# Rita-zi/WavTokenizer

Measured on AMD Instinct MI355X. Metric: audio-seconds/sec encode+decode, 24 kHz 3 s clips, higher is better.
Workload: dtype f32 (split-f16 x3 products)

## Files before the change

### include/wavtokenizer_amd.h

```cpp
#ifndef WAVTOKENIZER_AMD_H
#define WAVTOKENIZER_AMD_H

#include <stddef.h>
#include <stdint.h>

#ifdef __cplusplus
extern "C" {
#endif

typedef enum {
    WT_OK = 0,
    WT_ERR_INVALID = -1,
    WT_ERR_MISSING_TENSOR = -2,
    WT_ERR_SHAPE = -3,
    WT_ERR_HIP = -4,
    WT_ERR_NOT_INITED = -5,
    WT_ERR_RANGE = -6,
    WT_ERR_LSTM_SYNC = -7,
    WT_ERR_INDEX = -8
} wt_status;

enum wt_status_bits {
    WT_STATUS_BIT_LSTM = 1,
    WT_STATUS_BIT_RANGE = 2,
// ... 33 lines not shown
    WT_PLAN_DECODE_MIXED = 5,
    WT_PLAN_DECODE_CODES = 6,
    WT_PLAN_DECODE_CODES_MIXED = 7,
    WT_PLAN_QUANTIZE = 8
} wt_plan_kind;

enum {
    WT_PLAN_FLAG_KEEP_STAGES = 1,
    WT_PLAN_FLAG_UNFUSED = 16,
    WT_PLAN_FLAG_STEP_LSTM = 4,
    WT_PLAN_FLAG_GRAPH = 8,
    WT_PLAN_FLAG_FP32_GEMM = 2,
    WT_PLAN_FLAG_RANGE_REPORT = 32,
    WT_PLAN_FLAG_MIXED_LENGTH = 64,
    WT_PLAN_FLAG_F16_GEMM = 128,
    WT_PLAN_FLAG_RVQ = 256
};

enum wt_range_site {
    WT_SITE_ENCODER = 0,
    WT_SITE_BB_EMBED = 1,
    WT_SITE_RES0 = 2, WT_SITE_RES1 = 3,
    WT_SITE_ATTN = 4,
    WT_SITE_RES2 = 5, WT_SITE_RES3 = 6,
    WT_SITE_CNX0 = 7,
    WT_SITE_HEAD = 40,
    WT_SITE_SEANET_DECODER = 41
};

const char* wt_last_error(void);
// ... 140 lines not shown
    const float* R;
    const float* gamma;
    float* C;
    float* C2;
    uint32_t* status;
    const int32_t* mix_geom;
} wt_gemm_desc;
typedef struct {
    int32_t BM, BN, waves_m, waves_n, stages, ks, prod, staged, bias_cache, G, tiles;
} wt_launch_form;
size_t wt_gemm_probe_workspace_bytes(const wt_gemm_desc* d);
int wt_gemm_probe(const wt_gemm_desc* d, wt_launch_form* form, void* workspace, void* stream);

enum { WT_OP_GN_APPLY = 0, WT_OP_GN_STATS = 1, WT_OP_ROWNORM = 2, WT_OP_SOFTMAX = 3, WT_OP_ISTFT_OLA = 4, WT_OP_CONV_FIRST = 5,
       WT_OP_CONV_LAST = 6, WT_OP_TRANSPOSE = 7, WT_OP_CONVTR = 8, WT_OP_ROW_SUMSQ = 9, WT_OP_S32_AMAX = 10,
       WT_OP_CODE_ROWS = 12 };
enum { WT_OPK_GN_TILE = 1, WT_OPK_GN_CHUNK = 2, WT_OPK_GN_STATS = 3, WT_OPK_ROWNORM = 4, WT_OPK_DWCONV_LN = 5,
       WT_OPK_SOFTMAX_REG = 6, WT_OPK_SOFTMAX_RMW = 7, WT_OPK_ISTFT_OLA = 8, WT_OPK_CONV_FIRST = 9, WT_OPK_CONV_LAST32 = 10,
       WT_OPK_CONV_LAST = 11, WT_OPK_TRANSPOSE = 12, WT_OPK_CONVTR = 13, WT_OPK_ROW_SUMSQ = 14, WT_OPK_S32_AMAX = 15,
       WT_OPK_TRANSPOSE_MIXED = 16, WT_OPK_GN_MIXED = 17, WT_OPK_DWCONV_LN_MIXED = 18, WT_OPK_SOFTMAX_REG_MIXED = 19,
       WT_OPK_SOFTMAX_RMW_MIXED = 20, WT_OPK_ISTFT_OLA_MIXED = 21,
       WT_OPK_CODE_ROWS = 22, WT_OPK_CODE_ROWS_MIXED = 23 };
typedef struct {
    int32_t size;
    int32_t op;
    int32_t B, L, C;
    int32_t groups, mode, flag, out_s32;
    int32_t ld, k, stride, Cout, n_fft, hop, Kq;
    float eps;
    int64_t n;
    const void* x;
    const void *p0, *p1, *p2, *p3, *p4, *p5;
    void *y, *y2, *y3;
    uint32_t* status;
    const int32_t* lengths;
} wt_op_desc;
typedef struct {
// ... 248 lines not shown
```

### wavtokenizer_amd/_capi.py

```python
from __future__ import annotations

import ctypes
import os
from ctypes import POINTER, c_char_p, c_float, c_int32, c_int64, c_size_t, c_void_p

_HERE = os.path.dirname(os.path.abspath(__file__))
LIB_PATH = os.environ.get("WAVTOK_HIP_LIB") or os.path.join(_HERE, "libwavtok_hip.so")

EXPORTS = [
    "wt_last_error", "wt_version", "wt_model_create", "wt_model_destroy", "wt_model_export_bytes", "wt_model_export", "wt_packed_info", "wt_packed_verify", "wt_packed_bytes",
    "wt_model_create_packed", "wt_model_hop", "wt_model_weight_bytes",
    "wt_plan_create", "wt_plan_create_ex", "wt_plan_range_sites", "wt_plan_range_report", "wt_model_persistent_lstm", "wt_device_info", "wt_plan_destroy", "wt_plan_workspace_bytes", "wt_plan_frames", "wt_plan_num_launches", "wt_plan_graph_replays",
    "wt_plan_find_buffer", "wt_plan_buffer_info", "wt_plan_buffer_name", "wt_plan_status", "wt_plan_num_steps", "wt_plan_step_name",
    "wt_plan_set_timing", "wt_plan_read_timing", "wt_model_split_ok", "wt_model_status", "wt_model_take_bad_codes", "wt_encode", "wt_codes_to_features",
    "wt_decode", "wt_seanet_decode", "wt_head", "wt_unit_run", "wt_sconv1d", "wt_linear", "wt_conv1d_s32", "wt_vq_workspace_bytes",
    "wt_vq_nearest", "wt_vq_nearest_f32", "wt_resblock", "wt_resblock_down", "wt_gemm_probe_workspace_bytes", "wt_gemm_probe", "wt_op_probe",
    "wt_resampler_create", "wt_resampler_destroy", "wt_resampler_out_length", "wt_convert_audio", "wt_pcm16",
    "wt_linear_overlap_add", "wt_encode_mixed", "wt_plan_min_clip_length", "wt_sconv_geometry", "wt_decode_mixed",
    "wt_resblock_probe", "wt_geometry_words", "wt_geometry_probe", "wt_lstm_probe_workspace_bytes", "wt_lstm_probe",
    "wt_decode_codes", "wt_decode_codes_mixed", "wt_ingest_workspace_bytes", "wt_ingest", "wt_codes_unpack",
    "wt_emit_workspace_bytes", "wt_emit", "wt_vq_probe", "wt_overlap_add_ragged_workspace_bytes", "wt_overlap_add_ragged",
    "wt_model_weight_count", "wt_model_weight_info", "wt_split_probe",
    "wt_encode_rvq", "wt_encode_rvq_mixed", "wt_quantize", "wt_vq_residual_probe", "wt_model_codebook_tables",
    "wt_mel_create", "wt_mel_destroy", "wt_mel_frames", "wt_mel_tables", "wt_mel_workspace_bytes", "wt_mel_spectrogram", "wt_mel_distance",
# ... 4 lines not shown
]

WT_PLAN_ENCODE, WT_PLAN_DECODE, WT_PLAN_SEANET_DECODER, WT_PLAN_HEAD, WT_PLAN_UNIT_LSTM = 0, 1, 2, 3, 4
WT_PLAN_DECODE_MIXED = 5
WT_PLAN_DECODE_CODES, WT_PLAN_DECODE_CODES_MIXED = 6, 7
WT_PLAN_QUANTIZE = 8
WT_PLAN_FLAG_KEEP_STAGES = 1
WT_PLAN_FLAG_FP32_GEMM = 2
WT_PLAN_FLAG_F16_GEMM = 128
WT_PLAN_FLAG_STEP_LSTM = 4
WT_PLAN_FLAG_GRAPH = 8
WT_PLAN_FLAG_UNFUSED = 16
WT_PLAN_FLAG_RANGE_REPORT = 32
WT_PLAN_FLAG_MIXED_LENGTH = 64
WT_PLAN_FLAG_RVQ = 256
WT_SITE_ENCODER, WT_SITE_BB_EMBED, WT_SITE_RES0, WT_SITE_RES1, WT_SITE_ATTN, WT_SITE_RES2, WT_SITE_RES3 = 0, 1, 2, 3, 4, 5, 6
WT_SITE_CNX0, WT_SITE_HEAD, WT_SITE_SEANET_DECODER = 7, 40, 41
WT_ERR_INVALID = -1
WT_ERR_RANGE, WT_ERR_LSTM_SYNC, WT_ERR_INDEX = -6, -7, -8
WT_STATUS_BIT_LSTM, WT_STATUS_BIT_RANGE, WT_STATUS_BIT_LENGTH = 1, 2, 4
BUF_S32, BUF_ELU = 1, 2


class WtArch(ctypes.Structure):
    _fields_ = [("n_ratios", c_int32), ("ratios", c_int32 * 8), ("vq_bins", c_int32), ("num_quantizers", c_int32),
                ("input_channels", c_int32), ("dim", c_int32), ("intermediate_dim", c_int32),
                ("num_layers", c_int32), ("adanorm_num_embeddings", c_int32), ("n_fft", c_int32),
                ("hop_length", c_int32), ("padding_same", c_int32)]


# ... 7 lines not shown
                + [(n, c_int32) for n in ("T_in", "T_out", "Cin", "taps", "stride", "dil", "pad_left", "pad_mode", "Tp",
                                         "K1", "nz", "tap_pair", "head_kb")]
                + [("alpha", c_float)]
                + [(n, c_int64) for n in ("a_bstride", "a_rstride", "a2_bstride", "a2_rstride", "w_rstride", "c_rstride",
                                         "r_rstride", "zA", "zW", "zC")]
                + [(n, c_void_p) for n in ("A", "A2", "B", "bias", "R", "gamma", "C", "C2", "status", "mix_geom")])


class WtLaunchForm(ctypes.Structure):
    _fields_ = [(n, c_int32) for n in ("BM", "BN", "waves_m", "waves_n", "stages", "ks", "prod", "staged", "bias_cache", "G", "tiles")]


WT_OP_GN_APPLY, WT_OP_GN_STATS, WT_OP_ROWNORM, WT_OP_SOFTMAX, WT_OP_ISTFT_OLA, WT_OP_CONV_FIRST = 0, 1, 2, 3, 4, 5
WT_OP_CONV_LAST, WT_OP_TRANSPOSE, WT_OP_CONVTR, WT_OP_ROW_SUMSQ, WT_OP_S32_AMAX = 6, 7, 8, 9, 10
WT_OP_CODE_ROWS = 12
WT_OPK_NAMES = {1: "gn_tile", 2: "gn_chunk", 3: "gn_stats", 4: "rownorm", 5: "dwconv_ln", 6: "softmax_reg", 7: "softmax_rmw",
                8: "istft_ola", 9: "conv_first", 10: "conv_last32", 11: "conv_last", 12: "transpose", 13: "convtr",
                14: "row_sumsq", 15: "s32_amax", 16: "transpose_mixed", 17: "gn_mixed", 18: "dwconv_ln_mixed",
                19: "softmax_reg_mixed", 20: "softmax_rmw_mixed", 21: "istft_ola_mixed", 22: "code_rows", 23: "code_rows_mixed"}
WT_OPK_CODE_ROWS, WT_OPK_CODE_ROWS_MIXED = 22, 23


class WtOpDesc(ctypes.Structure):
    _fields_ = ([(n, c_int32) for n in ("size", "op", "B", "L", "C", "groups", "mode", "flag", "out_s32", "ld", "k", "stride",
                                        "Cout", "n_fft", "hop", "Kq")]
                + [("eps", c_float), ("n", c_int64)]
                + [(n, c_void_p) for n in ("x", "p0", "p1", "p2", "p3", "p4", "p5", "y", "y2", "y3", "status", "lengths")])


class WtOpForm(ctypes.Structure):
    _fields_ = [(n, c_int32) for n in ("kernel", "variant", "variant2", "grid_x", "grid_y", "grid_z", "block", "lds")]


class WtResblockDesc(ctypes.Structure):
    _fields_ = ([(n, c_int32) for n in ("size", "B", "T", "C", "r", "elu_out", "out_s32", "fp32_chain")]
# ... 308 lines not shown
```

### wavtokenizer_amd/csrc/capi.cpp

```cpp
#include "model.h"

namespace wt {
static thread_local std::string g_err;
void set_error(const std::string& msg) { g_err = msg; }
thread_local LaunchCtx g_launch;
int device_cus() {
    static std::atomic<int> cache[64];
    int d = 0;
    (void)hipGetDevice(&d);
    d &= 63;
    int v = cache[d].load(std::memory_order_relaxed);
    if (v <= 0) {
        if (hipDeviceGetAttribute(&v, hipDeviceAttributeMultiprocessorCount, d) != hipSuccess || v <= 0) v = 256;
        cache[d].store(v, std::memory_order_relaxed);
    }
    return v;
}
bool full_chip(int device) {
    int cus = 0;
    return hipDeviceGetAttribute(&cus, hipDeviceAttributeMultiprocessorCount, device) == hipSuccess && cus == 256;
}
}

using namespace wt;
// ... 195 lines not shown
    {WT_PLAN_UNIT_LSTM, build_unit_lstm, SITE_ENC, false, false},
    {WT_PLAN_DECODE_MIXED, build_decode, -1, true, false},
    {WT_PLAN_DECODE_CODES, build_decode, -1, true, false},  {WT_PLAN_DECODE_CODES_MIXED, build_decode, -1, true, false},
    {WT_PLAN_QUANTIZE, build_quantize, SITE_ENC, false, false},
};

int wt_plan_create_ex(const wt_model* m, int32_t kind, int32_t B, int64_t len, int32_t flags, uint64_t fp32_sites, wt_plan** out) {
    if (!m || !out) { set_error("wt_plan_create: null argument"); return WT_ERR_INVALID; }
    if (m->arch.num_layers > SITE_HEAD - SITE_CNX0) { set_error("wt_plan_create: more ConvNeXt blocks than range sites"); return WT_ERR_INVALID; }
    if (B < 1 || len < 1) { set_error("wt_plan_create: B and len must be >= 1"); return WT_ERR_INVALID; }
    if ((flags & WT_PLAN_FLAG_MIXED_LENGTH) && kind != WT_PLAN_ENCODE) {
        set_error("wt_plan_create: WT_PLAN_FLAG_MIXED_LENGTH is an encode-plan flag"); return WT_ERR_INVALID;
    }
    if ((flags & WT_PLAN_FLAG_RVQ) && kind != WT_PLAN_ENCODE) {
        set_error("wt_plan_create: WT_PLAN_FLAG_RVQ is an encode-plan flag (WT_PLAN_QUANTIZE runs the rounds on features)"); return WT_ERR_INVALID;
    }
    if (kind == WT_PLAN_QUANTIZE) {
        const struct { int flag; const char* name; } refused[] = {
            {WT_PLAN_FLAG_UNFUSED, "WT_PLAN_FLAG_UNFUSED"}, {WT_PLAN_FLAG_STEP_LSTM, "WT_PLAN_FLAG_STEP_LSTM"},
            {WT_PLAN_FLAG_MIXED_LENGTH, "WT_PLAN_FLAG_MIXED_LENGTH"}, {WT_PLAN_FLAG_F16_GEMM, "WT_PLAN_FLAG_F16_GEMM"}};
        for (const auto& r : refused)
            if (flags & r.flag) { set_error(std::string("wt_plan_create: ") + r.name + " has no meaning for WT_PLAN_QUANTIZE"); return WT_ERR_INVALID; }
    }
    if (flags & WT_PLAN_FLAG_F16_GEMM) {
        const bool decode_kind = kind == WT_PLAN_DECODE || kind == WT_PLAN_DECODE_MIXED || kind == WT_PLAN_DECODE_CODES ||
                                 kind == WT_PLAN_DECODE_CODES_MIXED;
        if (!decode_kind) { set_error("wt_plan_create: WT_PLAN_FLAG_F16_GEMM is a flag of the decode plan kinds"); return WT_ERR_INVALID; }
        if (flags & (WT_PLAN_FLAG_FP32_GEMM | WT_PLAN_FLAG_UNFUSED)) {
            set_error("wt_plan_create: WT_PLAN_FLAG_F16_GEMM does not combine with WT_PLAN_FLAG_FP32_GEMM or WT_PLAN_FLAG_UNFUSED");
            return WT_ERR_INVALID;
// ... 85 lines not shown
```

### wavtokenizer_amd/csrc/common.h

```cpp
#pragma once
#include <hip/hip_runtime.h>
#include <stdint.h>
#include <stdio.h>
#include <stdlib.h>
#include <mutex>
#include <string>

namespace wt {

void set_error(const std::string& msg);

#define WT_HIP_CHECK(expr)                                                                      \
    do {                                                                                        \
        hipError_t _e = (expr);                                                                 \
        if (_e != hipSuccess) {                                                                 \
            ::wt::set_error(std::string(#expr) + ": " + hipGetErrorString(_e));                 \
            return -4;                                                                          \
        }                                                                                       \
    } while (0)

struct PerDeviceOnce {
    std::mutex mu;
    bool seen[64] = {};
    template <class F> int run(F&& f) {
// ... 2 lines not shown
        d &= 63;
        std::lock_guard<std::mutex> g(mu);
        if (seen[d]) return 0;
        if (int rc = f()) return rc;
        seen[d] = true;
        return 0;
    }
};

enum : unsigned { WT_STATUS_LSTM = 1u, WT_STATUS_RANGE = 2u, WT_STATUS_LENGTH = 4u };
enum OpKernel : int {
    OPK_NONE = 0, OPK_GN_TILE, OPK_GN_CHUNK, OPK_GN_STATS, OPK_ROWNORM, OPK_DWCONV_LN, OPK_SOFTMAX_REG, OPK_SOFTMAX_RMW,
    OPK_ISTFT_OLA, OPK_CONV_FIRST, OPK_CONV_LAST32, OPK_CONV_LAST, OPK_TRANSPOSE, OPK_CONVTR, OPK_ROW_SUMSQ, OPK_S32_AMAX,
    OPK_TRANSPOSE_MIXED, OPK_GN_MIXED, OPK_DWCONV_LN_MIXED, OPK_SOFTMAX_REG_MIXED, OPK_SOFTMAX_RMW_MIXED, OPK_ISTFT_OLA_MIXED,
    OPK_CODE_ROWS, OPK_CODE_ROWS_MIXED,
    OPK_VQ_RESIDUAL
};
struct OpForm {
    int kernel = OPK_NONE;
    int variant = 0;
    int variant2 = 0;
    unsigned grid[3] = {0, 0, 0};
    unsigned block = 0;
    unsigned lds = 0;
};
struct RbForm {
    int kernel = -1;
    int C = 0, fold = 0, down = 0, fpw = 0;
    unsigned grid = 0, block = 0, lds = 0;
    long tiles = 0;
};
// ... 271 lines not shown
    unsigned* status;
    const float* Wd;
    const float* bd;
    float* y_down;
    int R;
};
struct ResblockMix {
    const int* T = nullptr;
    const int* Tread = nullptr;
};
bool resblock_fusable(int C);
int launch_resblock(const ResblockArgs& a, hipStream_t s);
int launch_resblock16(const ResblockArgs& a, hipStream_t s, const ResblockMix* mix = nullptr);
bool resblock16_down_fusable(int C, long T, int r, int k);
int launch_resblock16_down(const ResblockArgs& a, hipStream_t s, const ResblockMix* mix = nullptr);
int launch_mixed_geometry(const int* lengths, int* geom, int B, long Tpad, int tmin, int n_st, const int* kd, const int* rd,
                          int kf, hipStream_t s);
int launch_mixed_pad(const int* geom, int l_word, int64_t* codes, float* feat_ncl, float* emb_ncl, int B, int L, int D,
                     hipStream_t s);
int launch_mixed_check_lengths(const int* lengths, int B, int Lpad, unsigned* status, hipStream_t s);
int launch_convtr(const float* x, const float* w , const float* bias, float* y, int B, int Tin,
                  int Cin, int Cout, int k, int stride, int elu_in, hipStream_t s);

}
```

### wavtokenizer_amd/csrc/plan.cpp

```cpp
#include "model.h"

namespace wt {

static bool site_fp32(const wt_plan* P, int site) { return (P->fp32_sites >> site) & 1u; }
static bool plan_fp32(const wt_plan* P) {
    if ((P->flags & WT_PLAN_FLAG_FP32_GEMM) || !P->model->s32_ok) return true;
    if (P->whole_site == SITE_SEADEC && !P->model->sd_s32_ok) return true;
    return P->whole_site >= 0 && site_fp32(P, P->whole_site);
}
static bool plan_unfused(const wt_plan* P) { return P->flags & WT_PLAN_FLAG_UNFUSED; }
static bool plan_s32(const wt_plan* P) { return !plan_unfused(P) && !plan_fp32(P); }

static int gemm_auto(const wt_plan* P, const GemmArgs& a, int pro, int epi, hipStream_t s) {
    if (P->model->f32_stale.load()) if (int rc = ensure_f32_weights(P->model)) return rc;
    return launch_gemm(a, pro, epi, s);
}

static void set_s32(GemmArgs& a, const S32Copy& c) {
    a.W_hi = c.p; a.acc_scale = c.acc_scale; a.tap_pair = c.tap_pair ? 1 : 0;
}

static int gemm_s32(const GemmArgs& a, int epi, int out, hipStream_t s, const int* mix = nullptr, int prec = GEMM16S_F16X3) {
    if (!a.W_hi) { set_error("internal: no S32 copy of this weight"); return WT_ERR_INVALID; }
    return launch_gemm16s(a, epi, out, s, mix, prec);
// ... 184 lines not shown
    const int h = P->buf(name + ".h", (size_t)B * T * (C / 2), BUF_S32 | BUF_ELU);
    GemmArgs a3 = sconv_args(c3, B, T, 1, 1);
    GemmBufs b3{x_elu, -1, h};
    b3.x_off = x_off; b3.mix_word = mix_word >= 0 ? mix_word + GEOM_C3 : -1;
    if (x_bstride) a3.a_bstride = x_bstride;
    gemm_step(P, true, a3, b3, PRO_NONE, EPI_BIAS_ELU, OUT_S32);
    const int o = P->buf(name, (size_t)B * T * C, BUF_S32 | BUF_ELU);
    GemmArgs ac = sconv_args(sc, B, T, 1, 1);
    ac.W = cat.w; ac.w_rstride = cat.cin; ac.bias = cat.b; ac.K = cat.cin; ac.Cin = cat.cin;
    set_s32(ac, cat.s32);
    ac.K1 = C; ac.a2_bstride = T * (C / 2); ac.a2_rstride = C / 2;
    if (x_bstride) ac.a_bstride = x_bstride;
    GemmBufs bc{x_raw, h, o};
    bc.x_off = x_off; bc.mix_word = mix_word >= 0 ? mix_word + GEOM_SC : -1;
    gemm_step(P, true, ac, bc, PRO_NONE, EPI_BIAS_ELU, OUT_S32);
    return o;
}

static int plan_rvq_rounds(wt_plan* P, int x, int xs, bool s32, int geom, int l_word) {
    const wt_model* M = P->model;
    const int B = P->B, L = (int)P->L, bins = M->arch.vq_bins, D = M->embed.cols, nq = M->arch.num_quantizers;
    const long rows = (long)B * L;
    const int np = s32 ? gemm16s_vq_parts(bins) : gemm_vq_parts(bins);
    const int xx = P->buf("vq.xx", (size_t)rows);
    const int pv = P->buf("vq.pval", (size_t)rows * np);
    const int pi = P->buf("vq.pidx", (size_t)rows * np);
    const int r = nq > 1 ? P->buf("vq.r", (size_t)rows * D) : -1;
    const int rs = nq > 1 && s32 ? P->buf("vq.r.s32", (size_t)rows * D, BUF_S32) : -1;
    P->n_codes = rows;
    P->step({x, xx}, [=](const RunCtx& c) { return launch_row_sumsq(P->ptr(c, x), P->ptr(c, xx), rows, D, c.stream); });
// ... 57 lines not shown
    const long T = P->T;
    const bool rvq = P->flags & WT_PLAN_FLAG_RVQ;
    if (rvq) if (int rc = rvq_prepare(P)) return rc;
    const bool fold_e0 = !plan_unfused(P) && !M->stages.empty() && M->stages[0].C == 32 &&
                         M->e0_k == 7 && resblock_fusable(32);
    int x = -1;
    if (!fold_e0) {
        x = P->buf("enc.0", (size_t)B * T * M->e0_c);
        const int x0 = x;
        P->step({x0}, [=](const RunCtx& c) {
            return launch_conv_first(c.in_f, M->e0_w, M->e0_b, P->ptr(c, x0), B, T, M->e0_k, M->e0_c, c.stream);
        });
    }
    const bool fuse_elu = !plan_unfused(P);
    const bool s32 = plan_s32(P);
    struct Route { bool fused, down, s32; };
    std::vector<Route> route(M->stages.size());
    for (size_t si = 0; si < route.size(); ++si) {
        const ResStage& st = M->stages[si];
        Route& r = route[si];
        r.fused = resblock_fusable(st.C) && !plan_unfused(P);
        r.s32 = s32 && st.C % 32 == 0 && st.down.s32.p &&
                (r.fused || (si > 0 && route[si - 1].s32 && st.c3.s32.p && st.c1.s32.p && st.sc.s32.p));
        r.down = si == 0 && fold_e0 && r.fused && r.s32 && route.size() > 1 && resblock_fusable(M->stages[1].C) &&
                 st.down.cin == 32 && st.down.cout == 64 && resblock16_down_fusable(st.C, T, st.r, st.down.k);
    }
    const bool lstm_s32 = !route.empty() && route.back().s32 && M->enc_lstm.Wih0.s32.p;
    const bool tail_s32 = lstm_s32 && M->enc_final.s32.p && M->embed.s32.p;
    const bool mixed = P->flags & WT_PLAN_FLAG_MIXED_LENGTH;
    const int n_st = (int)route.size();
    int geom = -1;
    if (mixed) {
        bool ok = s32 && !(P->flags & (WT_PLAN_FLAG_KEEP_STAGES | WT_PLAN_FLAG_RANGE_REPORT)) && tail_s32 &&
                  n_st >= 2 && n_st <= GEOM_MAX_STAGES && route[0].down;
        for (int si = 1; si < n_st && ok; ++si)
            ok = route[si].s32 && (route[si].fused ? M->stages[si].C == 64 : M->stages[si].cat.s32.p != nullptr);
        for (const ResStage& st : M->stages) ok = ok && st.c3.k == 3 && st.sc.k == 1;
        if (!ok) {
            set_error("mixed-length plans run only the shipped split-f16 encoder route: not with WT_PLAN_FLAG_UNFUSED, "
                      "FP32_GEMM, KEEP_STAGES or RANGE_REPORT, an encoder range site on fp32, or weights without S32 copies");
// ... 31 lines not shown
                if (geom >= 0) { mix.T = mix_ptr(c, GEOM_T); mix.Tread = mix_ptr(c, GEOM_TREAD); }
                a.wav = c.in_f; a.e0_w = M->e0_w; a.e0_b = M->e0_b;
                a.W3 = st.c3.w; a.b3 = st.c3.b; a.W1 = st.c1.w; a.b1 = st.c1.b; a.Ws = st.sc.w; a.bs = st.sc.b;
                a.Wd = st.down.w; a.bd = st.down.b; a.y_down = P->ptr(c, y); a.R = st.r;
                a.B = B; a.T = (int)Tc; a.C = st.C;
                return launch_resblock16_down(a, c.stream, geom >= 0 ? &mix : nullptr);
            }, 1, "resblock.fused_down");
            x = y; Tc = ad.T_out; idx += 3;
            continue;
        }
        const std::string name = "enc." + std::to_string(idx);
        const int stage_word = GEOM_STAGE0 + (int)si * GEOM_STAGE_WORDS;
        if (r.fused)
            x = plan_resblock(P, st.c3, st.c1, st.sc, B, Tc, x, name, fuse_elu, (si == 0 && fold_e0) ? M : nullptr, 0, 0, r.s32,
                              mixed ? stage_word + GEOM_C3 : -1);
        else if (r.s32)
            x = plan_resblock_s32(P, st.c3, st.sc, st.cat, B, Tc, x, x_elu, name, 0, 0, mixed ? stage_word : -1);
        else
            x = plan_resblock(P, st.c3, st.c1, st.sc, B, Tc, x, name, fuse_elu);
        if (x < 0) return WT_ERR_INVALID;
        const bool next_s32 = !last && !route[si + 1].fused && route[si + 1].s32;
        const int y = P->buf(out, ynum, next_s32 ? BUF_S32 : BUF_F32);
        const int y2 = (next_s32 || (last && lstm_s32)) ? P->buf(out + ".s32", ynum, BUF_S32 | (next_s32 ? BUF_ELU : 0)) : -1;
        GemmBufs bd{x, -1, y, y2};
        bd.mix_word = mixed ? stage_word + GEOM_DOWN : -1;
        gemm_step(P, r.s32, ad, bd, fuse_elu ? PRO_NONE : PRO_ELU, EPI_BIAS,
                  next_s32 ? OUT_S32_DUAL_ELU : (y2 >= 0 ? OUT_F32_AND_S32 : OUT_F32));
        if (next_s32) x_elu = y2;
        if (last) x_s32 = y2;
        x = y; Tc = ad.T_out; idx += 3;
    }
    const int L = (int)Tc;
    if (L != P->L) { set_error("internal: frame count mismatch"); return WT_ERR_INVALID; }
    P->n_codes = (long)B * L; P->n_out = P->n_aux = (long)B * 512 * L;
    const int H = M->H;
    x = plan_lstm(P, M->enc_lstm, B, L, H, x, "enc." + std::to_string(idx), fuse_elu, x_s32, tail_s32);
// ... 340 lines not shown
```

### wavtokenizer_amd/csrc/probe.cpp

```cpp
#include "model.h"

using namespace wt;

extern "C" {

int wt_codes_to_features(const wt_model* m, const int64_t* codes, int32_t K, int32_t B, int64_t L, float* features,
                         void* stream) {
    if (!m || !codes || !features) { set_error("wt_codes_to_features: null argument"); return WT_ERR_INVALID; }
    if (K < 1 || K > m->arch.num_quantizers) { set_error("wt_codes_to_features: K exceeds the number of codebooks"); return WT_ERR_INVALID; }
    DeviceGuard dg(m->device);
    if (!dg.ok) { set_error("hipSetDevice failed"); return WT_ERR_HIP; }
    return launch_codes_to_features(codes, m->embed.w, K, m->arch.vq_bins, B, L, 512, features, static_cast<hipStream_t>(stream),
                                    m->bad_codes_dev);
}

int wt_sconv1d(const float* x, const float* w, const float* bias, float* y, int32_t B, int64_t T, int32_t Cin,
               int32_t Cout, int32_t k, int32_t stride, int32_t dilation, int32_t elu_input, void* stream) {
    ConvW cw; cw.w = const_cast<float*>(w); cw.b = const_cast<float*>(bias); cw.cout = Cout; cw.cin = Cin; cw.k = k;
    GemmArgs a = sconv_args(cw, B, T, stride, dilation);
    a.A = x; a.C = y;
    return launch_gemm(a, elu_input ? PRO_ELU : PRO_NONE, EPI_BIAS, static_cast<hipStream_t>(stream));
}

static int split_pair(const float* w, long nw, const float* x, long nx, char* ws_w, char* ws_x, char* tail, GemmArgs& a,
// ... 143 lines not shown
    if (form) *form = wt_launch_form{lf.BM, lf.BN, lf.waves_m, lf.waves_n, lf.stages, lf.ks, lf.prod, lf.staged, lf.bias_cache, lf.G, lf.tiles};
    return WT_OK;
}

static int op_probe_check(const wt_op_desc* d) {
    auto bad = [](const char* m) { set_error(std::string("wt_op_probe: ") + m); return (int)WT_ERR_INVALID; };
    if (!d || (d->size != (int32_t)sizeof(wt_op_desc) && d->size != (int32_t)offsetof(wt_op_desc, lengths))) return bad("descriptor missing or of another size");
    const int32_t* lengths = d->size == (int32_t)sizeof(wt_op_desc) ? d->lengths : nullptr;
    if (lengths) {
        if (reinterpret_cast<uintptr_t>(lengths) & 3) return bad("lengths misaligned");
        const bool aware = d->op == WT_OP_GN_APPLY || d->op == WT_OP_GN_STATS || (d->op == WT_OP_ROWNORM && d->mode == RN_DWCONV) ||
                           d->op == WT_OP_SOFTMAX || d->op == WT_OP_ISTFT_OLA || d->op == WT_OP_TRANSPOSE || d->op == WT_OP_CODE_ROWS;
        if (!aware) return bad("this op has no length-aware launch");
        if (d->op == WT_OP_SOFTMAX && (d->L <= 0 || d->n % d->L)) return bad("the length-aware softmax needs whole clips of L rows");
    }
    if (d->op < WT_OP_GN_APPLY || (d->op > WT_OP_S32_AMAX && d->op != WT_OP_CODE_ROWS)) return bad("unknown op");
    auto al16 = [](const void* p) { return !(reinterpret_cast<uintptr_t>(p) & 15); };
    const void* ptrs[] = {d->p0, d->p1, d->p2, d->p3, d->p4, d->p5, d->y, d->y2, d->y3};
    for (const void* p : ptrs) if (!al16(p)) return bad("arrays must be 16-byte aligned");
    if (!d->x || (reinterpret_cast<uintptr_t>(d->x) & (d->op == WT_OP_SOFTMAX ? 3 : 15))) return bad("x missing or misaligned");
    if (reinterpret_cast<uintptr_t>(d->status) & 3) return bad("status misaligned");
    const bool shaped = d->op != WT_OP_SOFTMAX && d->op != WT_OP_ROW_SUMSQ && d->op != WT_OP_S32_AMAX;
    if (shaped && (d->B <= 0 || d->L <= 0)) return bad("extents must be positive");
    if (shaped && d->op != WT_OP_CONV_FIRST && d->op != WT_OP_ISTFT_OLA && (d->C <= 0 || (long)d->L * d->C >= (long)INT_MAX)) return bad("extents must be positive (and L * C < 2^31)");
    switch (d->op) {
    case WT_OP_GN_APPLY: case WT_OP_GN_STATS:
        if (!d->p0 || !d->p1 || !d->y2 || !d->y3 || (d->op == WT_OP_GN_APPLY && !d->y)) return bad("null argument");
        if (d->groups <= 0 || d->C % d->groups || d->C / d->groups > 256 || d->B > 65535) return bad("GroupNorm needs C % groups == 0, at most 256 channels per group, B <= 65535");
        break;
    case WT_OP_ROWNORM:
        if (!d->y || !d->p4 || !d->p5) return bad("null argument");
// ... 28 lines not shown
    case WT_OP_ROW_SUMSQ:
        if (!d->y) return bad("null argument");
        if (d->n <= 0 || d->C <= 0 || d->C % 4) return bad("row_sumsq needs rows > 0 and C % 4 == 0");
        break;
    case WT_OP_S32_AMAX:
        if (!d->y) return bad("null argument");
        if (d->n <= 0 || d->n % 32) return bad("s32_amax needs whole S32 groups of 32 values");
        break;
    case WT_OP_CODE_ROWS:
        if (!d->p0 || !d->y) return bad("null argument");
        if (d->k < 1 || d->n < 1 || d->n > INT_MAX) return bad("code_rows needs k >= 1 codebooks of 1 <= n < 2^31 bins");
        if (d->C % 4 || d->C > 1024) return bad("code_rows needs C % 4 == 0 and C <= 1024");
        if (d->out_s32 && d->C % 32) return bad("code_rows: an S32 output needs C % 32 == 0");
        if ((long)d->B * d->L >= (long)INT_MAX) return bad("code_rows: too many frames for one launch");
        break;
    }
    return WT_OK;
}

int wt_op_probe(const wt_op_desc* d, wt_op_form* form, void* stream) {
    if (int rc = op_probe_check(d)) return rc;
    hipStream_t s = static_cast<hipStream_t>(stream);
    auto F = [](const void* p) { return static_cast<const float*>(p); };
    auto W = [](void* p) { return static_cast<float*>(p); };
    OpForm lf;
    const int* lens = d->size == (int32_t)sizeof(wt_op_desc) ? d->lengths : nullptr;
    const LaunchCtx saved = g_launch;
    g_launch.status = reinterpret_cast<unsigned*>(d->status);
    g_launch.form = &lf;
    int rc = 0;
// ... 25 lines not shown
        rc = launch_transpose(F(d->x), W(d->y), d->B, d->L, d->C, s, d->out_s32 ? 1 : 0, lens);
        break;
    case WT_OP_CONVTR:
        rc = launch_convtr(F(d->x), F(d->p0), F(d->p1), W(d->y), d->B, d->L, d->C, d->Cout, d->k, d->stride, d->flag ? 1 : 0, s);
        break;
    case WT_OP_ROW_SUMSQ:
        rc = launch_row_sumsq(F(d->x), W(d->y), d->n, d->C, s);
        break;
    case WT_OP_S32_AMAX:
        rc = launch_s32_amax(d->x, d->n, static_cast<unsigned*>(d->y), s);
        break;
    case WT_OP_CODE_ROWS:
        rc = launch_code_rows(static_cast<const int64_t*>(d->x), F(d->p0), d->k, (int)d->n, d->B, d->L, d->C, W(d->y), s, d->out_s32 ? 1 : 0,
                              static_cast<unsigned*>(d->y2), lens);
        break;
    }
    g_launch = saved;
    if (rc) return rc;
    if (form) *form = wt_op_form{lf.kernel, lf.variant, lf.variant2, (int32_t)lf.grid[0], (int32_t)lf.grid[1], (int32_t)lf.grid[2], (int32_t)lf.block, (int32_t)lf.lds};
    return WT_OK;
}

size_t wt_vq_workspace_bytes(int64_t N, int32_t D, int32_t bins) {
    const size_t np = std::max(gemm_vq_parts(bins), gemm16s_vq_parts(bins));
    return al256((size_t)N * D * 4) + al256((size_t)bins * D * 4) + al256((size_t)N * sizeof(float)) +
           2 * al256((size_t)N * np * sizeof(float)) + al256((size_t)bins * sizeof(float)) + 512;
}

struct VqLayout { char *xs, *es; float* xx; float* pv; int* pi; float* ee; char* tail; int np; };
static VqLayout vq_layout(void* workspace, int64_t N, int32_t D, int32_t bins, bool s32) {
// ... 266 lines not shown
```

Measured before the change: 38210.

## Fuse the 128-channel encoder residual block into one persistent MFMA kernel

Adds a persistent kernel for the 128-channel encoder stage. In one launch it computes the k=3 conv to a 64-wide hidden, then the concatenated 1x1 shortcut-plus-projection GEMM, with ELU, bias and split-f16 handling kept in LDS. Four waves keep conv weights in registers and four waves keep the concat weights, so the intermediate activations never go to global memory. It also prefetches the next tile while the current one computes. The old multi-GEMM s32 path stays available through a new STAGE3_GEMM flag and is still used for mixed-length and range-report plans. The cost is one block per CU with high register and LDS use, which limits occupancy.

```diff
diff --git a/include/wavtokenizer_amd.h b/include/wavtokenizer_amd.h
--- a/include/wavtokenizer_amd.h
+++ b/include/wavtokenizer_amd.h
@@ -71,6 +71,7 @@
     WT_PLAN_FLAG_RANGE_REPORT = 32,
     WT_PLAN_FLAG_MIXED_LENGTH = 64,
     WT_PLAN_FLAG_F16_GEMM = 128,
+    WT_PLAN_FLAG_STAGE3_GEMM = 512,
     WT_PLAN_FLAG_RVQ = 256
 };
 
@@ -241,13 +242,15 @@
 
 enum { WT_OP_GN_APPLY = 0, WT_OP_GN_STATS = 1, WT_OP_ROWNORM = 2, WT_OP_SOFTMAX = 3, WT_OP_ISTFT_OLA = 4, WT_OP_CONV_FIRST = 5,
        WT_OP_CONV_LAST = 6, WT_OP_TRANSPOSE = 7, WT_OP_CONVTR = 8, WT_OP_ROW_SUMSQ = 9, WT_OP_S32_AMAX = 10,
-       WT_OP_CODE_ROWS = 12 };
+       WT_OP_CODE_ROWS = 12,
+       WT_OP_RESBLOCK128 = 13 };
 enum { WT_OPK_GN_TILE = 1, WT_OPK_GN_CHUNK = 2, WT_OPK_GN_STATS = 3, WT_OPK_ROWNORM = 4, WT_OPK_DWCONV_LN = 5,
        WT_OPK_SOFTMAX_REG = 6, WT_OPK_SOFTMAX_RMW = 7, WT_OPK_ISTFT_OLA = 8, WT_OPK_CONV_FIRST = 9, WT_OPK_CONV_LAST32 = 10,
        WT_OPK_CONV_LAST = 11, WT_OPK_TRANSPOSE = 12, WT_OPK_CONVTR = 13, WT_OPK_ROW_SUMSQ = 14, WT_OPK_S32_AMAX = 15,
        WT_OPK_TRANSPOSE_MIXED = 16, WT_OPK_GN_MIXED = 17, WT_OPK_DWCONV_LN_MIXED = 18, WT_OPK_SOFTMAX_REG_MIXED = 19,
        WT_OPK_SOFTMAX_RMW_MIXED = 20, WT_OPK_ISTFT_OLA_MIXED = 21,
-       WT_OPK_CODE_ROWS = 22, WT_OPK_CODE_ROWS_MIXED = 23 };
+       WT_OPK_CODE_ROWS = 22, WT_OPK_CODE_ROWS_MIXED = 23,
+       WT_OPK_RESBLOCK128 = 25 };
 typedef struct {
     int32_t size;
     int32_t op;
diff --git a/wavtokenizer_amd/_capi.py b/wavtokenizer_amd/_capi.py
--- a/wavtokenizer_amd/_capi.py
+++ b/wavtokenizer_amd/_capi.py
@@ -42,6 +42,7 @@
 WT_PLAN_FLAG_RANGE_REPORT = 32
 WT_PLAN_FLAG_MIXED_LENGTH = 64
 WT_PLAN_FLAG_RVQ = 256
+WT_PLAN_FLAG_STAGE3_GEMM = 512
 WT_SITE_ENCODER, WT_SITE_BB_EMBED, WT_SITE_RES0, WT_SITE_RES1, WT_SITE_ATTN, WT_SITE_RES2, WT_SITE_RES3 = 0, 1, 2, 3, 4, 5, 6
 WT_SITE_CNX0, WT_SITE_HEAD, WT_SITE_SEANET_DECODER = 7, 40, 41
 WT_ERR_INVALID = -1
@@ -79,11 +80,14 @@
 WT_OP_GN_APPLY, WT_OP_GN_STATS, WT_OP_ROWNORM, WT_OP_SOFTMAX, WT_OP_ISTFT_OLA, WT_OP_CONV_FIRST = 0, 1, 2, 3, 4, 5
 WT_OP_CONV_LAST, WT_OP_TRANSPOSE, WT_OP_CONVTR, WT_OP_ROW_SUMSQ, WT_OP_S32_AMAX = 6, 7, 8, 9, 10
 WT_OP_CODE_ROWS = 12
+WT_OP_RESBLOCK128 = 13
 WT_OPK_NAMES = {1: "gn_tile", 2: "gn_chunk", 3: "gn_stats", 4: "rownorm", 5: "dwconv_ln", 6: "softmax_reg", 7: "softmax_rmw",
                 8: "istft_ola", 9: "conv_first", 10: "conv_last32", 11: "conv_last", 12: "transpose", 13: "convtr",
                 14: "row_sumsq", 15: "s32_amax", 16: "transpose_mixed", 17: "gn_mixed", 18: "dwconv_ln_mixed",
-                19: "softmax_reg_mixed", 20: "softmax_rmw_mixed", 21: "istft_ola_mixed", 22: "code_rows", 23: "code_rows_mixed"}
+                19: "softmax_reg_mixed", 20: "softmax_rmw_mixed", 21: "istft_ola_mixed", 22: "code_rows", 23: "code_rows_mixed",
+                25: "resblock128"}
 WT_OPK_CODE_ROWS, WT_OPK_CODE_ROWS_MIXED = 22, 23
+WT_OPK_RESBLOCK128 = 25
 
 
 class WtOpDesc(ctypes.Structure):
diff --git a/wavtokenizer_amd/csrc/capi.cpp b/wavtokenizer_amd/csrc/capi.cpp
--- a/wavtokenizer_amd/csrc/capi.cpp
+++ b/wavtokenizer_amd/csrc/capi.cpp
@@ -233,6 +233,9 @@
     }
     if ((flags & WT_PLAN_FLAG_RVQ) && kind != WT_PLAN_ENCODE) {
         set_error("wt_plan_create: WT_PLAN_FLAG_RVQ is an encode-plan flag (WT_PLAN_QUANTIZE runs the rounds on features)"); return WT_ERR_INVALID;
+    }
+    if ((flags & WT_PLAN_FLAG_STAGE3_GEMM) && kind != WT_PLAN_ENCODE) {
+        set_error("wt_plan_create: WT_PLAN_FLAG_STAGE3_GEMM is an encode-plan flag"); return WT_ERR_INVALID;
     }
     if (kind == WT_PLAN_QUANTIZE) {
         const struct { int flag; const char* name; } refused[] = {
diff --git a/wavtokenizer_amd/csrc/common.h b/wavtokenizer_amd/csrc/common.h
--- a/wavtokenizer_amd/csrc/common.h
+++ b/wavtokenizer_amd/csrc/common.h
@@ -40,7 +40,8 @@
     OPK_ISTFT_OLA, OPK_CONV_FIRST, OPK_CONV_LAST32, OPK_CONV_LAST, OPK_TRANSPOSE, OPK_CONVTR, OPK_ROW_SUMSQ, OPK_S32_AMAX,
     OPK_TRANSPOSE_MIXED, OPK_GN_MIXED, OPK_DWCONV_LN_MIXED, OPK_SOFTMAX_REG_MIXED, OPK_SOFTMAX_RMW_MIXED, OPK_ISTFT_OLA_MIXED,
     OPK_CODE_ROWS, OPK_CODE_ROWS_MIXED,
-    OPK_VQ_RESIDUAL
+    OPK_VQ_RESIDUAL,
+    OPK_RESBLOCK128
 };
 struct OpForm {
     int kernel = OPK_NONE;
@@ -342,6 +343,20 @@
 int launch_resblock16(const ResblockArgs& a, hipStream_t s, const ResblockMix* mix = nullptr);
 bool resblock16_down_fusable(int C, long T, int r, int k);
 int launch_resblock16_down(const ResblockArgs& a, hipStream_t s, const ResblockMix* mix = nullptr);
+struct Resblock128Args {
+    const float* x;
+    const void* W3;
+    const void* Wc;
+    const float* b3;
+    const float* bc;
+    float* y;
+    int B, T;
+    float acc3, accc;
+    const float* acc_dev;
+    unsigned* status;
+};
+bool resblock128_fusable(int C, int k3, int ks);
+int launch_resblock128(const Resblock128Args& a, hipStream_t s);
 int launch_mixed_geometry(const int* lengths, int* geom, int B, long Tpad, int tmin, int n_st, const int* kd, const int* rd,
                           int kf, hipStream_t s);
 int launch_mixed_pad(const int* geom, int l_word, int64_t* codes, float* feat_ncl, float* emb_ncl, int B, int L, int D,
diff --git a/wavtokenizer_amd/csrc/plan.cpp b/wavtokenizer_amd/csrc/plan.cpp
--- a/wavtokenizer_amd/csrc/plan.cpp
+++ b/wavtokenizer_amd/csrc/plan.cpp
@@ -222,6 +222,20 @@
     GemmBufs bc{x_raw, h, o};
     bc.x_off = x_off; bc.mix_word = mix_word >= 0 ? mix_word + GEOM_SC : -1;
     gemm_step(P, true, ac, bc, PRO_NONE, EPI_BIAS_ELU, OUT_S32);
+    return o;
+}
+
+static int plan_resblock128(wt_plan* P, const ResStage& st, int B, long T, int xin, const std::string& name) {
+    const int o = P->buf(name, (size_t)B * T * st.C, BUF_S32 | BUF_ELU);
+    const ConvW c3 = st.c3, cat = st.cat;
+    P->step({xin, o}, [=](const RunCtx& c) {
+        Resblock128Args a{};
+        a.x = P->ptr(c, xin); a.y = P->ptr(c, o);
+        a.W3 = c3.s32.p; a.b3 = c3.b; a.acc3 = c3.s32.acc_scale;
+        a.Wc = cat.s32.p; a.bc = cat.b; a.accc = cat.s32.acc_scale;
+        a.B = B; a.T = (int)T;
+        return launch_resblock128(a, c.stream);
+    }, 1, "resblock.fused128");
     return o;
 }
 
@@ -309,7 +323,7 @@
     }
     const bool fuse_elu = !plan_unfused(P);
     const bool s32 = plan_s32(P);
-    struct Route { bool fused, down, s32; };
+    struct Route { bool fused, down, s32, f128; };
     std::vector<Route> route(M->stages.size());
     for (size_t si = 0; si < route.size(); ++si) {
         const ResStage& st = M->stages[si];
@@ -319,6 +333,9 @@
                 (r.fused || (si > 0 && route[si - 1].s32 && st.c3.s32.p && st.c1.s32.p && st.sc.s32.p));
         r.down = si == 0 && fold_e0 && r.fused && r.s32 && route.size() > 1 && resblock_fusable(M->stages[1].C) &&
                  st.down.cin == 32 && st.down.cout == 64 && resblock16_down_fusable(st.C, T, st.r, st.down.k);
+        r.f128 = !(P->flags & WT_PLAN_FLAG_STAGE3_GEMM) && si > 0 && !r.fused && r.s32 && resblock128_fusable(st.C, st.c3.k, st.sc.k) &&
+                 st.cat.s32.p && !st.c3.s32.tap_pair && !st.cat.s32.tap_pair &&
+                 !(P->flags & (WT_PLAN_FLAG_MIXED_LENGTH | WT_PLAN_FLAG_RANGE_REPORT));
     }
     const bool lstm_s32 = !route.empty() && route.back().s32 && M->enc_lstm.Wih0.s32.p;
     const bool tail_s32 = lstm_s32 && M->enc_final.s32.p && M->embed.s32.p;
@@ -380,12 +397,14 @@
         if (r.fused)
             x = plan_resblock(P, st.c3, st.c1, st.sc, B, Tc, x, name, fuse_elu, (si == 0 && fold_e0) ? M : nullptr, 0, 0, r.s32,
                               mixed ? stage_word + GEOM_C3 : -1);
+        else if (r.f128)
+            x = plan_resblock128(P, st, B, Tc, x, name);
         else if (r.s32)
             x = plan_resblock_s32(P, st.c3, st.sc, st.cat, B, Tc, x, x_elu, name, 0, 0, mixed ? stage_word : -1);
         else
             x = plan_resblock(P, st.c3, st.c1, st.sc, B, Tc, x, name, fuse_elu);
         if (x < 0) return WT_ERR_INVALID;
-        const bool next_s32 = !last && !route[si + 1].fused && route[si + 1].s32;
+        const bool next_s32 = !last && !route[si + 1].fused && route[si + 1].s32 && !route[si + 1].f128;
         const int y = P->buf(out, ynum, next_s32 ? BUF_S32 : BUF_F32);
         const int y2 = (next_s32 || (last && lstm_s32)) ? P->buf(out + ".s32", ynum, BUF_S32 | (next_s32 ? BUF_ELU : 0)) : -1;
         GemmBufs bd{x, -1, y, y2};
diff --git a/wavtokenizer_amd/csrc/probe.cpp b/wavtokenizer_amd/csrc/probe.cpp
--- a/wavtokenizer_amd/csrc/probe.cpp
+++ b/wavtokenizer_amd/csrc/probe.cpp
@@ -181,7 +181,7 @@
         if (!aware) return bad("this op has no length-aware launch");
         if (d->op == WT_OP_SOFTMAX && (d->L <= 0 || d->n % d->L)) return bad("the length-aware softmax needs whole clips of L rows");
     }
-    if (d->op < WT_OP_GN_APPLY || (d->op > WT_OP_S32_AMAX && d->op != WT_OP_CODE_ROWS)) return bad("unknown op");
+    if (d->op < WT_OP_GN_APPLY || (d->op > WT_OP_S32_AMAX && d->op != WT_OP_CODE_ROWS && d->op != WT_OP_RESBLOCK128)) return bad("unknown op");
     auto al16 = [](const void* p) { return !(reinterpret_cast<uintptr_t>(p) & 15); };
     const void* ptrs[] = {d->p0, d->p1, d->p2, d->p3, d->p4, d->p5, d->y, d->y2, d->y3};
     for (const void* p : ptrs) if (!al16(p)) return bad("arrays must be 16-byte aligned");
@@ -240,6 +240,11 @@
         if (d->out_s32 && d->C % 32) return bad("code_rows: an S32 output needs C % 32 == 0");
         if ((long)d->B * d->L >= (long)INT_MAX) return bad("code_rows: too many frames for one launch");
         break;
+    case WT_OP_RESBLOCK128:
+        if (!d->p0 || !d->p1 || !d->p2 || !d->p3 || !d->p4 || !d->y) return bad("null argument");
+        if (d->C != 128) return bad("resblock128 is the 128-channel block");
+        if ((long)d->B * d->L >= (long)INT_MAX / 64) return bad("resblock128: too many frames for one launch");
+        break;
     }
     return WT_OK;
 }
@@ -295,6 +300,13 @@
         rc = launch_code_rows(static_cast<const int64_t*>(d->x), F(d->p0), d->k, (int)d->n, d->B, d->L, d->C, W(d->y), s, d->out_s32 ? 1 : 0,
                               static_cast<unsigned*>(d->y2), lens);
         break;
+    case WT_OP_RESBLOCK128: {
+        Resblock128Args a{};
+        a.x = F(d->x); a.W3 = d->p0; a.b3 = F(d->p1); a.Wc = d->p2; a.bc = F(d->p3); a.acc_dev = F(d->p4); a.y = W(d->y);
+        a.B = d->B; a.T = d->L; a.acc3 = a.accc = 1.f;
+        rc = launch_resblock128(a, s);
+        break;
+    }
     }
     g_launch = saved;
     if (rc) return rc;
diff --git a/wavtokenizer_amd/csrc/resblock128.hip b/wavtokenizer_amd/csrc/resblock128.hip
--- /dev/null
+++ b/wavtokenizer_amd/csrc/resblock128.hip
@@ -0,0 +1,249 @@
+#include "common.h"
+
+namespace wt {
+
+typedef float f32x4 __attribute__((ext_vector_type(4)));
+typedef _Float16 f16x8 __attribute__((ext_vector_type(8)));
+typedef _Float16 f16x4 __attribute__((ext_vector_type(4)));
+
+namespace rb128 {
+constexpr int C = 128, H = 64, FT = 64, NX = FT + 2, NT = 512;
+constexpr int XB = C * 4, HB = H * 4;
+constexpr int off_xe = 0;
+constexpr int off_xr = off_xe + NX * XB;
+constexpr int off_he = off_xr + FT * XB;
+constexpr int off_yo = off_he + FT * HB;
+constexpr int total = off_yo + FT * XB;
+constexpr int ITEMS = (NX * (C / 4) + NT - 1) / NT;
+__device__ __forceinline__ int row_off(int r, int chunk, int bytes) { return r * bytes + ((chunk ^ (r & 15)) * 16); }
+__device__ __forceinline__ int hi_chunk(int n) { return (n >> 5) * 8 + ((n & 31) >> 3); }
+}
+
+__global__ __launch_bounds__(512, 1) void resblock128_kernel(const Resblock128Args a) {
+    using namespace rb128;
+    extern __shared__ __attribute__((aligned(256))) char smem128[];
+    char* xe = smem128 + off_xe;
+    char* xr = smem128 + off_xr;
+    char* he = smem128 + off_he;
+    char* yo = smem128 + off_yo;
+    const int tid = threadIdx.x;
+    const int wave = __builtin_amdgcn_readfirstlane(tid >> 6);
+    const bool cat_role = wave >= 4;
+    const int wr = wave & 3;
+
+    f16x8 wh[12], wl[12];
+    f32x4 bv[2];
+    {
+    const int m16 = tid & 15, q = (tid & 63) >> 4;
+    if (!cat_role) {
+        const char* p3 = reinterpret_cast<const char*>(a.W3) + (long)(16 * wr + m16) * (3 * C * 4) + q * 16;
+#pragma unroll
+        for (int s = 0; s < 12; ++s) {
+            wh[s] = *reinterpret_cast<const f16x8*>(p3 + s * 128);
+            wl[s] = *reinterpret_cast<const f16x8*>(p3 + s * 128 + 64);
+        }
+        bv[0] = *reinterpret_cast<const f32x4*>(a.b3 + 16 * wr + 4 * q);
+        bv[1] = bv[0];
+    } else {
+#pragma unroll
+        for (int rt = 0; rt < 2; ++rt) {
+            const char* pc = reinterpret_cast<const char*>(a.Wc) + (long)(32 * wr + 16 * rt + m16) * ((C + H) * 4) + q * 16;
+#pragma unroll
+            for (int s = 0; s < 6; ++s) {
+                wh[6 * rt + s] = *reinterpret_cast<const f16x8*>(pc + s * 128);
+                wl[6 * rt + s] = *reinterpret_cast<const f16x8*>(pc + s * 128 + 64);
+            }
+            bv[rt] = *reinterpret_cast<const f32x4*>(a.bc + 32 * wr + 16 * rt + 4 * q);
+        }
+    }
+    }
+    const float acc3 = a.acc_dev ? a.acc_dev[0] : a.acc3, accc = a.acc_dev ? a.acc_dev[1] : a.accc;
+    const float acc_s = cat_role ? accc : acc3;
+    const float lo_s = acc_s * (1.f / 2048.f);
+
+    const int tiles_per_clip = (a.T + FT - 1) / FT;
+    const long n_tiles = (long)a.B * tiles_per_clip;
+    const int Tp = a.T > 1 ? a.T : 2;
+    float amax = 0.f;
+
+    auto finish = [&](const f32x4 m, const f32x4 c, const f32x4 bias, bool valid, f16x4& hi, f16x4& lo) {
+        f32x4 v;
+        v.x = fmaf(c.x, lo_s, m.x * acc_s);
+        v.y = fmaf(c.y, lo_s, m.y * acc_s);
+        v.z = fmaf(c.z, lo_s, m.z * acc_s);
+        v.w = fmaf(c.w, lo_s, m.w * acc_s);
+        v = v + bias;
+        v.x = elu_med3(v.x); v.y = elu_med3(v.y); v.z = elu_med3(v.z); v.w = elu_med3(v.w);
+        if (valid) amax = amax4(amax, v.x, v.y, v.z, v.w);
+        split4_f16(v.x, v.y, v.z, v.w, hi, lo);
+    };
+
+    f32x4 px[ITEMS];
+    auto prefetch = [&](long tile, int tv) {
+        const int b = (int)(tile / tiles_per_clip), t0 = (int)(tile % tiles_per_clip) * FT;
+#pragma unroll
+        for (int it = 0; it < ITEMS; ++it) {
+            const int e = tv + it * NT;
+            const int r = e >> 5, c4 = (e & 31) * 4;
+            int pos = t0 - 1 + r;
+            pos = pos < 0 ? -pos : pos;
+            pos = pos >= Tp ? 2 * (Tp - 1) - pos : pos;
+            f32x4 v = {0.f, 0.f, 0.f, 0.f};
+            if (e < NX * (C / 4) && pos >= 0 && pos < a.T)
+                v = *reinterpret_cast<const f32x4*>(a.x + ((long)b * a.T + pos) * C + c4);
+            px[it] = v;
+        }
+    };
+    if ((long)blockIdx.x < n_tiles) prefetch(blockIdx.x, tid);
+
+    for (long tile = blockIdx.x; tile < n_tiles; tile += gridDim.x) {
+        const int b = (int)(tile / tiles_per_clip), t0 = (int)(tile % tiles_per_clip) * FT;
+        int tv = tid;
+        asm volatile("" : "+v"(tv));
+        const int m16 = tv & 15, q = (tv & 63) >> 4, lane = tv & 63;
+        auto frag_off = [&](int rl, int bytes, int j) { return rl * bytes + ((((j << 2) | q) ^ (rl & 15)) * 16); };
+        auto run_off = [&](int fr, int n, int bytes, int lo) { return row_off(fr, hi_chunk(n) + 4 * lo, bytes) + (n & 7) * 2; };
+#pragma unroll
+        for (int it = 0; it < ITEMS; ++it) {
+            const int e = tv + it * NT;
+            if (e < NX * (C / 4)) {
+                const int r = e >> 5, c4 = (e & 31) * 4;
+                const int ch = hi_chunk(c4), sub = (c4 & 7) * 2;
+                const f32x4 v = px[it];
+                f16x4 hi, lo;
+                if (r >= 1 && r <= FT) {
+                    const f32x4 vr = t0 - 1 + r < a.T ? v : f32x4{0.f, 0.f, 0.f, 0.f};
+                    amax = amax4(amax, vr.x, vr.y, vr.z, vr.w);
+                    split4_f16(vr.x, vr.y, vr.z, vr.w, hi, lo);
+                    *reinterpret_cast<f16x4*>(xr + row_off(r - 1, ch, XB) + sub) = hi;
+                    *reinterpret_cast<f16x4*>(xr + row_off(r - 1, ch + 4, XB) + sub) = lo;
+                }
+                split4_f16(elu_med3(v.x), elu_med3(v.y), elu_med3(v.z), elu_med3(v.w), hi, lo);
+                *reinterpret_cast<f16x4*>(xe + row_off(r, ch, XB) + sub) = hi;
+                *reinterpret_cast<f16x4*>(xe + row_off(r, ch + 4, XB) + sub) = lo;
+            }
+        }
+        __syncthreads();
+        if (tile + gridDim.x < n_tiles) prefetch(tile + gridDim.x, tv);
+
+        if (!cat_role) {
+            f32x4 hm[4], hc[4];
+#pragma unroll
+            for (int ct = 0; ct < 4; ++ct) { hm[ct] = f32x4{0.f, 0.f, 0.f, 0.f}; hc[ct] = hm[ct]; }
+#pragma unroll
+            for (int s = 0; s < 12; ++s) {
+                const int tap = s >> 2, g = s & 3;
+                const char* ph = xe + frag_off(m16 + tap, XB, 2 * (g & 1)) + (g >> 1) * 256;
+                const char* pl = xe + frag_off(m16 + tap, XB, 2 * (g & 1) + 1) + (g >> 1) * 256;
+                f16x8 bh[4], bl[4];
+#pragma unroll
+                for (int ct = 0; ct < 4; ++ct) {
+                    bh[ct] = *reinterpret_cast<const f16x8*>(ph + ct * 16 * XB);
+                    bl[ct] = *reinterpret_cast<const f16x8*>(pl + ct * 16 * XB);
+                }
+#pragma unroll
+                for (int ct = 0; ct < 4; ++ct) {
+                    hm[ct] = __builtin_amdgcn_mfma_f32_16x16x32_f16(wh[s], bh[ct], hm[ct], 0, 0, 0);
+                    hc[ct] = __builtin_amdgcn_mfma_f32_16x16x32_f16(wl[s], bh[ct], hc[ct], 0, 0, 0);
+                }
+#pragma unroll
+                for (int ct = 0; ct < 4; ++ct) hc[ct] = __builtin_amdgcn_mfma_f32_16x16x32_f16(wh[s], bl[ct], hc[ct], 0, 0, 0);
+            }
+            const int n = 16 * wr + 4 * q;
+#pragma unroll
+            for (int ct = 0; ct < 4; ++ct) {
+                const int fr = 16 * ct + m16;
+                f16x4 hi, lo;
+                finish(hm[ct], hc[ct], bv[0], t0 + fr < a.T, hi, lo);
+                *reinterpret_cast<f16x4*>(he + run_off(fr, n, HB, 0)) = hi;
+                *reinterpret_cast<f16x4*>(he + run_off(fr, n, HB, 1)) = lo;
+            }
+            __syncthreads();
+        } else {
+            f32x4 ym[2][4], yc[2][4];
+#pragma unroll
+            for (int rt = 0; rt < 2; ++rt)
+#pragma unroll
+                for (int ct = 0; ct < 4; ++ct) { ym[rt][ct] = f32x4{0.f, 0.f, 0.f, 0.f}; yc[rt][ct] = ym[rt][ct]; }
+            auto k_step = [&](int s, const char* ph, const char* pl, int ct_bytes) {
+#pragma unroll
+                for (int cp = 0; cp < 2; ++cp) {
+                    f16x8 bh[2], bl[2];
+#pragma unroll
+                    for (int c = 0; c < 2; ++c) {
+                        bh[c] = *reinterpret_cast<const f16x8*>(ph + (2 * cp + c) * ct_bytes);
+                        bl[c] = *reinterpret_cast<const f16x8*>(pl + (2 * cp + c) * ct_bytes);
+                    }
+#pragma unroll
+                    for (int rt = 0; rt < 2; ++rt)
+#pragma unroll
+                        for (int c = 0; c < 2; ++c) {
+                            ym[rt][2 * cp + c] = __builtin_amdgcn_mfma_f32_16x16x32_f16(wh[6 * rt + s], bh[c], ym[rt][2 * cp + c], 0, 0, 0);
+                            yc[rt][2 * cp + c] = __builtin_amdgcn_mfma_f32_16x16x32_f16(wl[6 * rt + s], bh[c], yc[rt][2 * cp + c], 0, 0, 0);
+                        }
+#pragma unroll
+                    for (int rt = 0; rt < 2; ++rt)
+#pragma unroll
+                        for (int c = 0; c < 2; ++c)
+                            yc[rt][2 * cp + c] = __builtin_amdgcn_mfma_f32_16x16x32_f16(wh[6 * rt + s], bl[c], yc[rt][2 * cp + c], 0, 0, 0);
+                }
+            };
+#pragma unroll
+            for (int s = 0; s < 4; ++s)
+                k_step(s, xr + frag_off(m16, XB, 2 * (s & 1)) + (s >> 1) * 256, xr + frag_off(m16, XB, 2 * (s & 1) + 1) + (s >> 1) * 256, 16 * XB);
+            __syncthreads();
+#pragma unroll
+            for (int s = 4; s < 6; ++s)
+                k_step(s, he + frag_off(m16, HB, 2 * (s & 1)), he + frag_off(m16, HB, 2 * (s & 1) + 1), 16 * HB);
+#pragma unroll
+            for (int rt = 0; rt < 2; ++rt) {
+                const int n = 32 * wr + 16 * rt + 4 * q;
+#pragma unroll
+                for (int ct = 0; ct < 4; ++ct) {
+                    const int fr = 16 * ct + m16;
+                    f16x4 hi, lo;
+                    finish(ym[rt][ct], yc[rt][ct], bv[rt], t0 + fr < a.T, hi, lo);
+                    *reinterpret_cast<f16x4*>(yo + run_off(fr, n, XB, 0)) = hi;
+                    *reinterpret_cast<f16x4*>(yo + run_off(fr, n, XB, 1)) = lo;
+                }
+            }
+        }
+        __syncthreads();
+
+#pragma unroll
+        for (int it = 0; it < 4; ++it) {
+            const int r = 8 * wave + 2 * it + (lane >> 5), ch = lane & 31;
+            const f32x4 v = *reinterpret_cast<const f32x4*>(yo + row_off(r, ch, XB));
+            if (t0 + r < a.T) *reinterpret_cast<f32x4*>(a.y + ((long)b * a.T + t0 + r) * C + ch * 4) = v;
+        }
+    }
+    range_report(a.status, amax);
+}
+
+bool resblock128_fusable(int C, int k3, int ks) { return C == rb128::C && k3 == 3 && ks == 1; }
+
+int launch_resblock128(const Resblock128Args& a, hipStream_t s) {
+    auto al16 = [](const void* p) { return p && !(reinterpret_cast<uintptr_t>(p) & 15); };
+    if (!al16(a.x) || !al16(a.W3) || !al16(a.Wc) || !al16(a.b3) || !al16(a.bc) || !al16(a.y)) {
+        set_error("resblock128: arrays missing or not 16-byte aligned"); return -1;
+    }
+    if (a.B < 1 || a.T < 1 || (long)a.B * a.T >= (long)INT32_MAX / rb128::FT) { set_error("resblock128: extents out of range"); return -1; }
+    static PerDeviceOnce attr_once;
+    constexpr size_t smem = (size_t)rb128::total;
+    static_assert(smem <= 160 * 1024, "LDS budget");
+    if (int rc = attr_once.run([&]() -> int {
+        WT_HIP_CHECK(hipFuncSetAttribute(reinterpret_cast<const void*>(resblock128_kernel), hipFuncAttributeMaxDynamicSharedMemorySize, (int)smem));
+        return 0;
+    })) return rc;
+    const long tiles = (long)a.B * ((a.T + rb128::FT - 1) / rb128::FT);
+    const long slots = device_cus();
+    const long grid = tiles < slots ? tiles : slots;
+    Resblock128Args b = a;
+    if (!b.status) b.status = g_launch.status;
+    if (OpForm* f = g_launch.form) *f = OpForm{OPK_RESBLOCK128, (int)tiles, 0, {(unsigned)grid, 1u, 1u}, (unsigned)rb128::NT, (unsigned)smem};
+    hipLaunchKernelGGL(resblock128_kernel, dim3((unsigned)grid), dim3(rb128::NT), smem, s, b);
+    WT_HIP_CHECK(hipGetLastError());
+    return 0;
+}
+
+}
```

New measurement: 38310, median of 3. About the same (+0.3%).
